# cs2mosa/Heterogeneous-MOE-for-Diffusion-models

Measured on AMD Instinct MI355X. Metric: denoise-steps/sec (fwd+bwd) on 4x32x32 latents, higher is better.
Workload: dtype bf16

## Files before the change

heterogeneous-moe-for-diffusion-models_amd/csrc/pbwd.hip:

```cpp
#include "common.h"
#include "conv_args.h"
#include "hdmoe.h"

namespace {

struct PbwArgs {
  const bf16* x; const bf16* dy; const bf16* wd; bf16* dx; float* G[HDMOE_MAX_GROUPS]; const int* seg;
  int ngroups, N, I, O, upw;
  long HW, wdstride;
  float alpha;
};
typedef __attribute__((ext_vector_type(4))) short s16x4;
typedef __attribute__((address_space(3))) s16x4* lds_p4;

DEVI bool pbw_slot(const PbwArgs& a, int slot, int& g, long& p0, long& p1, long& u0, long& u1) {
  for (g = 0; g < a.ngroups; ++g) {
    const long r0 = a.seg ? a.seg[g] : 0, r1 = a.seg ? a.seg[g + 1] : a.N;
    p0 = r0 * a.HW; p1 = r1 * a.HW;
    const long units = p1 > p0 ? (p1 - p0 + 63) >> 6 : 0;
    const long nch = (units + a.upw - 1) / a.upw;
    if (slot < nch) { u0 = (long)slot * a.upw; u1 = u0 + a.upw < units ? u0 + a.upw : units; return true; }
    slot -= (int)nch;
  }
  return false;
}

template <int OT, int IT>
__global__ __launch_bounds__(256) void pw_bwd_kernel(PbwArgs a) {
  constexpr int WB = (OT + IT) * 4096, T = OT * IT;
  extern __shared__ __attribute__((aligned(1024))) unsigned char lds[];
  const int tid = threadIdx.x, lane = tid & 63, wave = tid >> 6;
  int g; long p0, p1, u0, u1;
  if (!pbw_slot(a, blockIdx.x, g, p0, p1, u0, u1)) return;
  const bf16* X = a.x;
  const bf16* DY = a.dy;
  bf16* DX = a.dx;
  unsigned char* mine = lds + wave * WB;
  const int r = lane & 31, h = lane >> 5;
  bf16x8 wfr[IT][OT][2];
  {
    const bf16* WD = a.wd + (long)g * a.wdstride;
#pragma unroll
    for (int u = 0; u < IT; ++u)
#pragma unroll
      for (int t = 0; t < OT; ++t)
#pragma unroll
        for (int k2 = 0; k2 < 2; ++k2) wfr[u][t][k2] = *reinterpret_cast<const bf16x8*>(WD + (long)(32 * u + r) * a.O + 32 * t + 16 * k2 + 8 * h);
  }
  uint4 sdy[4 * OT], sx[4 * IT];
  auto load = [&](long u) {
    const long pb = p0 + (u << 6);
#pragma unroll
    for (int k = 0; k < 4 * OT; ++k) {
      const int e = lane + 64 * k, q = e / (4 * OT), pc = e % (4 * OT);
      const long p = pb + q;
      sdy[k] = *reinterpret_cast<const uint4*>(DY + (p < p1 ? p : p0) * a.O + pc * 8);
    }
#pragma unroll
    for (int k = 0; k < 4 * IT; ++k) {
      const int e = lane + 64 * k, q = e / (4 * IT), pc = e % (4 * IT);
      const long p = pb + q;
      sx[k] = *reinterpret_cast<const uint4*>(X + (p < p1 ? p : p0) * a.I + pc * 8);
    }
#pragma unroll
    for (int k = 0; k < 4 * OT; ++k) if (pb + (lane + 64 * k) / (4 * OT) >= p1) sdy[k] = make_uint4(0, 0, 0, 0);
#pragma unroll
    for (int k = 0; k < 4 * IT; ++k) if (pb + (lane + 64 * k) / (4 * IT) >= p1) sx[k] = make_uint4(0, 0, 0, 0);
  };
  auto store = [&]() {
#pragma unroll
    for (int k = 0; k < 4 * OT; ++k) {
      const int e = lane + 64 * k, q = e / (4 * OT), pc = e % (4 * OT);
      *reinterpret_cast<uint4*>(mine + (pc >> 2) * 4096 + q * 64 + (pc & 3) * 16) = sdy[k];
    }
#pragma unroll
    for (int k = 0; k < 4 * IT; ++k) {
      const int e = lane + 64 * k, q = e / (4 * IT), pc = e % (4 * IT);
      *reinterpret_cast<uint4*>(mine + OT * 4096 + (pc >> 2) * 4096 + q * 64 + (pc & 3) * 16) = sx[k];
    }
  };
  const int q4 = (lane & 15) >> 2, col4 = (lane & 16) + 4 * (lane & 3);
  const int tlane = (8 * h + q4) * 64 + col4 * 2;
  auto tr2 = [&](const unsigned char* base) -> bf16x8 {
    const s16x4 lo = __builtin_amdgcn_ds_read_tr16_b64_v4i16((lds_p4)(base));
    const s16x4 hi = __builtin_amdgcn_ds_read_tr16_b64_v4i16((lds_p4)(base + 4 * 64));
    return __builtin_bit_cast(bf16x8, __builtin_shufflevector(lo, hi, 0, 1, 2, 3, 4, 5, 6, 7));
  };
  f32x16 acc[OT][IT];
#pragma unroll
  for (int t = 0; t < OT; ++t)
#pragma unroll
    for (int u = 0; u < IT; ++u) acc[t][u] = (f32x16)(0.f);
  auto wfence = [&]() {
    __builtin_amdgcn_fence(__ATOMIC_RELEASE, "wavefront");
    __builtin_amdgcn_wave_barrier();
    __builtin_amdgcn_fence(__ATOMIC_ACQUIRE, "wavefront");
  };
  const long iters = (u1 - u0 + 3) >> 2;
  if (u0 + wave < u1) load(u0 + wave);
  for (long it = 0; it < iters; ++it) {
    const long u = u0 + wave + 4 * it;
    const bool valid = u < u1;
    wfence();
    if (valid) store();
    wfence();
    if (u + 4 < u1) load(u + 4);
    if (valid) {
#pragma unroll
      for (int ks = 0; ks < 4; ++ks) {
        bf16x8 fdy[OT], fx[IT];
#pragma unroll
        for (int t = 0; t < OT; ++t) fdy[t] = tr2(mine + t * 4096 + ks * 1024 + tlane);
#pragma unroll
        for (int v = 0; v < IT; ++v) fx[v] = tr2(mine + (OT + v) * 4096 + ks * 1024 + tlane);
#pragma unroll
        for (int t = 0; t < OT; ++t)
#pragma unroll
          for (int v = 0; v < IT; ++v) acc[t][v] = __builtin_amdgcn_mfma_f32_32x32x16_bf16(fdy[t], fx[v], acc[t][v], 0, 0, 0);
      }
      wfence();
#pragma unroll
      for (int hh = 0; hh < 2; ++hh) {
        f32x16 ax[IT];
#pragma unroll
        for (int v = 0; v < IT; ++v) ax[v] = (f32x16)(0.f);
#pragma unroll
        for (int t = 0; t < OT; ++t)
#pragma unroll
          for (int k2 = 0; k2 < 2; ++k2) {
            const bf16x8 d = *reinterpret_cast<const bf16x8*>(mine + t * 4096 + (32 * hh + r) * 64 + (2 * k2 + h) * 16);
#pragma unroll
            for (int v = 0; v < IT; ++v) ax[v] = __builtin_amdgcn_mfma_f32_32x32x16_bf16(wfr[v][t][k2], d, ax[v], 0, 0, 0);
          }
#pragma unroll
        for (int v = 0; v < IT; ++v)
#pragma unroll
          for (int q = 0; q < 4; ++q) {
            bf16x4 o4;
#pragma unroll
            for (int j = 0; j < 4; ++j) o4[j] = (bf16)(a.alpha * ax[v][4 * q + j]);
            *reinterpret_cast<bf16x4*>(mine + (OT + v) * 4096 + (32 * hh + r) * 64 + (8 * q + 4 * h) * 2) = o4;
          }
      }
      wfence();
      const long pb = p0 + (u << 6);
#pragma unroll
      for (int k = 0; k < 4 * IT; ++k) {
        const int e = lane + 64 * k, q = e / (4 * IT), pc = e % (4 * IT);
        const uint4 v = *reinterpret_cast<const uint4*>(mine + OT * 4096 + (pc >> 2) * 4096 + q * 64 + (pc & 3) * 16);
        if (pb + q < p1) *reinterpret_cast<uint4*>(DX + (pb + q) * a.I + pc * 8) = v;
      }
    }
  }
  float* red = reinterpret_cast<float*>(lds);
  auto put = [&](int s) {
#pragma unroll
    for (int t = 0; t < OT; ++t)
#pragma unroll
      for (int v = 0; v < IT; ++v)
#pragma unroll
        for (int reg = 0; reg < 16; ++reg) red[((s * T + t * IT + v) * 16 + reg) * 64 + lane] = acc[t][v][reg];
  };
  __syncthreads();
  if (wave >= 2) put(wave - 2);
  __syncthreads();
  if (wave < 2) {
#pragma unroll
    for (int t = 0; t < OT; ++t)
#pragma unroll
      for (int v = 0; v < IT; ++v)
#pragma unroll
        for (int reg = 0; reg < 16; ++reg) acc[t][v][reg] += red[((wave * T + t * IT + v) * 16 + reg) * 64 + lane];
  }
  __syncthreads();
  if (wave < 2) put(wave);
  __syncthreads();
  float* G = a.G[g];
  const int rot = (int)((blockIdx.x * 17u) % (unsigned)(T * 4)) * 256;
  for (int e0 = tid; e0 < T * 1024; e0 += 256) {
    const int e = (e0 + rot) % (T * 1024);
    const int l = e & 63, reg = (e >> 6) & 15, tu = e >> 10;
    const float v = red[(tu * 16 + reg) * 64 + l] + red[((T + tu) * 16 + reg) * 64 + l];
    const int o = 32 * (tu / IT) + acc_row(reg, l), i = 32 * (tu % IT) + (l & 31);
    atomicAdd(&G[(long)o * a.I + i], v);
  }
}

template <int OT, int IT>
int pbw_launch(const PbwArgs& a, unsigned slots, size_t lds, hipStream_t stream) {
  static unsigned long long attr = 0;
  if (hdmoe_first_on_device(attr)) { (void)hipFuncSetAttribute((const void*)pw_bwd_kernel<OT, IT>, hipFuncAttributeMaxDynamicSharedMemorySize, 160 * 1024); }
  hipLaunchKernelGGL((pw_bwd_kernel<OT, IT>), dim3(slots), dim3(256), lds, stream, a);
  return hdmoe_launch_status();
}

}

extern "C" int hdmoe_pw_bwd(const void* x, const void* dy, const void* wd, void* dx, float* const* G, const int* seg, int ngroups,
                            long wd_stride, int N, long HW, int Cin, int Cout, float alpha, int dtype, hipStream_t stream) {
  if (dtype != HDMOE_BF16 || Cin < 32 || Cout < 32 || Cin % 32 || Cout % 32 || Cin > 128 || Cout > 128) return 1;
  const int OT = Cout / 32, IT = Cin / 32;
  if (OT * IT > 8) return 1;
  if (!x || !dy || !wd || !dx || !G || ngroups < 1 || ngroups > HDMOE_MAX_GROUPS || N < 0 || HW < 0) return HDMOE_EINVAL;
  if ((((uintptr_t)x | (uintptr_t)dy | (uintptr_t)wd | (uintptr_t)dx) & 15) || wd_stride % 8 || wd_stride < (long)Cin * Cout) return 1;
  const long total = (long)N * HW;
  if (total == 0) return HDMOE_OK;
  if (total >= (1l << 40)) return 1;
  PbwArgs a;
  a.x = (const bf16*)x; a.dy = (const bf16*)dy; a.wd = (const bf16*)wd; a.dx = (bf16*)dx; a.seg = seg;
  a.ngroups = ngroups; a.N = N; a.HW = HW; a.I = Cin; a.O = Cout; a.wdstride = wd_stride; a.alpha = alpha;
  for (int g = 0; g < HDMOE_MAX_GROUPS; ++g) {
    a.G[g] = G[g < ngroups ? g : 0];
    if (!a.G[g]) return HDMOE_EINVAL;
  }
  const size_t stage = (size_t)4 * (OT + IT) * 4096, red = (size_t)2 * OT * IT * 4096;
  const size_t lds = stage > red ? stage : red;
  const long target = OT + IT <= 3 ? 512 : 256;
  const long units = (total + 63) / 64 + ngroups;
  long upw = (units + target - 1) / target;
  upw = (upw + 3) / 4 * 4;
  if (upw > (1l << 24)) return 1;
  a.upw = (int)upw;
  const long slots = units / upw + ngroups + 1;
  if (slots >= (1l << 31)) return 1;
  hdmoe_count_selection(HDMOE_SEL_PW_BWD);
  int rc = 1;
  conv_pick<1, 2, 3, 4>(OT, [&](auto Ot) { conv_pick<1, 2, 3, 4>(IT, [&](auto It) {
    constexpr int O = decltype(Ot)::value, I = decltype(It)::value;
    if constexpr (O * I <= 8) rc = pbw_launch<O, I>(a, (unsigned)slots, lds, stream);
  }); });
  return rc;
}
```

heterogeneous-moe-for-diffusion-models_amd/hdmoe_hip/ops.py:

```python
from __future__ import annotations

import ctypes
import functools
import math
from typing import Optional, Sequence, Tuple, Union

import torch

from . import bank as _bank
from ._lib import dtype_code_cast
from ._lib import BF16, _int_array, call, dtype_code, lib

Tensor = torch.Tensor

F32S = 2
ROUTE_CONV6S = 6


def _c(t: Optional[Tensor]) -> Optional[Tensor]:
    if t is None:
        return None
    return t if t.is_contiguous() else t.contiguous()


# ... 325 lines not shown
        return _fused_bwd(bank, ent, self.label, self.name, x, dy, ent.wd, dx, self.mid, ws, self.tail, self.defer, self.stats)


def _kxk_bwd_plan(L: _ConvLayer, seg, policy: str, stats: tuple, kernel: str, film: bool = False, gn_in=(None, None, 0)) -> _BwdPlan:
    geom, defer = (L.N, L.H, L.W, L.I, L.O, L.khs, L.kws, L.pts, L.pts, L.alpha), (seg, L.G, L.N, L.H, L.W, L.I, L.O, L.dtc, L.khs)
    if L.dtc != F32S:
        return _BwdPlan("hdmoe_conv_bwd6", L.dtc, policy, (seg, L.G, L.wdstride, *geom), (L.dtc,), defer, stats,
                        lambda: L.record(seg, 2.0, name=kernel, dtype="bfloat16"), film)
    return _BwdPlan("hdmoe_conv_bwd6s", F32S, policy, (seg, L.G, L.wdstride, L.G * L.wdstride, *geom), (*gn_in, 1 if TRUNK_BWD_BF16 else 0), defer, stats,
                    lambda: L.record(seg, 2.0, name=kernel, dtype="bfloat16" if TRUNK_BWD_BF16 else "split_bf16"))


def _conv_bwd_plan(L: _ConvLayer, seg, need_dx: bool, ones6: bool, device) -> Optional[_BwdPlan]:
    same = not L.ones and L.Ho == L.H and L.Wo == L.W and L.Cphys == L.I
    conv6 = need_dx and _prof_ok() and same and L.khs == L.kws
    if conv6 and L.dtc == BF16 and set(L.khs) == {3, 5}:
        return _kxk_bwd_plan(L, seg, "arena", ("bwd6",), "bwd6_kernel", film=True)
    if conv6 and L.split and set(L.khs) == {3}:
        return _kxk_bwd_plan(L, seg, "arena", ("bwd6s",), "bwd6s_kernel")
    if ones6:
        def scratch():
            S = torch.empty((L.G, L.H, L.W, L.O), dtype=torch.float32, device=device)
            g32 = [_zeros((kh * kw, L.O, L.Cphys), torch.float32, device) for kh, kw in zip(L.khs, L.kws)]
            return (S, g32, seg, L.G, L.wdstride, L.N, L.H, L.W, L.Cphys, L.O, L.Opad, L.khs, L.alpha)
        return _BwdPlan("hdmoe_conv6_ones_bwd", L.dtc, "stream", scratch, (L.dtc,), None, (),
                        lambda: L.record(seg, 2.0 if need_dx else 1.0, name="conv6 dgrad + wgrad6 (ones-channel layer)", dtype="bfloat16"))
    if need_dx and _prof_ok() and same and L.dtc == BF16 and all(k == 1 for k in L.khs + L.kws):
        return _BwdPlan("hdmoe_pw_bwd", L.dtc, None, (seg, L.G, L.wdstride, L.N, L.H * L.W, L.I, L.O, L.alpha), (L.dtc,), None, ("pbwd",),
                        lambda: L.record(seg, 2.0, name="pw_bwd_kernel", dtype="bfloat16"))
    return None


def _fused_bwd(bank, ent, label, name, x, dy, wd, dx, mid, ws, tail, defer, stats) -> bool:
    wsargs = () if ws is None else (ws, ws.numel() * 4)
    if _timed("fused", label, name, x, dy, wd, dx, list(ent.G), *mid, *wsargs, *tail) != 0:
        return False
    if defer is not None:
        seg, *shape = defer
        bank.defer_w6(ent.G, seg, ws, *shape, ent=ent)
    else:
        bank.note_backward(ent)
    for k in stats:
        STATS[k] += 1
    return True


def _wgrad(x, dy, Gs, seg, G, N, H, W, Ho, Wo, I, Cphys, O, ones, khs, kws, pts, split=False, bank=None):
    def rec(w6=None):
        if w6:
            return lambda: _conv_record(x, seg, N, Ho * Wo, O, I, khs, kws, "split_bf16" if split else None, wgrad_name=w6)
        return lambda: _conv_record(x, seg, N, Ho * Wo, O, I, khs, kws, wgrad_name=_kernel_label(_route(
            "hdmoe_conv_wgrad_route", 34, N, H, W, Ho, Wo, I, Cphys, O, 1, ones, G, seg is not None, khs, kws, pts, pts, _dt(x),
            x.data_ptr() % 16 == 0 and dy.data_ptr() % 16 == 0), x, wgrad=True))
    w6 = "wgrad6_kernel<split>" if split else "wgrad6_kernel"
    if (x.dtype == torch.bfloat16 or split) and not ones and Ho == H and Wo == W and Cphys == I:
        dtc = F32S if split else _dt(x)
        kib = _w6_kib(G, N, H, W, I, O, khs, kws, dtc)
        ws = _w6_workspace("arena", x.device, kib) if bank is not None and _prof_ok() else None
        if ws is not None:
            if _timed("conv_wgrad", rec(w6 + " (deferred reduce)"), "hdmoe_conv_wgrad6", x, dy, Gs, seg, G, N, H, W, I, O, khs, kws, pts, pts, ws, ws.numel() * 4,
                      dtc, 1) == 0:
                bank.defer_w6(Gs, seg, ws, G, N, H, W, I, O, dtc, khs)
                STATS["w6_defer"] += 1
                return
        ws = _w6_workspace("stream", x.device, kib)
        if ws is not None:
            if _timed("conv_wgrad", rec(w6 + " (+ reduce)"), "hdmoe_conv_wgrad6", x, dy, Gs, seg, G, N, H, W, I, O, khs, kws, pts, pts, ws, ws.numel() * 4, dtc, 0) == 0:
                return
    _timed("conv_wgrad", rec(), "hdmoe_conv_wgrad", x, dy, Gs, seg, G, N, H, W, Ho, Wo, I, Cphys, O, 1, 1 if ones else 0, khs, kws, pts, pts, _dt(x))


_ConvCall = _collections.namedtuple("_ConvCall", "G gain_val alpha beta ones training normalize split res_raw out film")


class _MPConvFn(torch.autograd.Function):

    @staticmethod
    def forward(ctx, x, res, seg, c: _ConvCall, *tensors):
        G, gain_val, alpha, beta, ones, training, normalize, split = c.G, c.gain_val, c.alpha, c.beta, c.ones, c.training, c.normalize, c.split
        weights, gains = tensors[:G], list(tensors[G:]) or None
        ctx.film = getattr(x, "_film_rec", None) if FILM_DGRAD and x.is_contiguous() else None
        if ctx.film is not None:
            ctx.film.register()
        x = _c(x)
        N, H, W, Cphys = x.shape
        O, I = int(weights[0].shape[0]), int(weights[0].shape[1])
        khs = [_kernel_hw(w)[0] for w in weights]
        kws = [_kernel_hw(w)[1] for w in weights]
        pts = [(kw - 1) // 2 for kw in kws]
        Hos = {H + (kw - 1) - kh + 1 for kh, kw in zip(khs, kws)}
        if len(Hos) != 1:
            raise ValueError("grouped conv: all groups must produce the same output size")
        if any(w.shape[0] != O or w.shape[1] != I for w in weights):
            raise ValueError("grouped conv: all groups must share (out_channels, in_channels)")
        if I != Cphys + (1 if ones else 0):
            raise RuntimeError(f"MP_Conv: input has {Cphys} channels, weight expects {I}")
        Ho, Wo = Hos.pop(), W
        Ipad = (I + 15) // 16 * 16
        Opad = (O + 15) // 16 * 16
        taps = max(a * b for a, b in zip(khs, kws))
        wstride, wdstride = taps * O * Ipad, taps * I * Opad
        wdt, planes, dtc = (torch.bfloat16, 2, F32S) if split else (x.dtype, 1, _dt(x))
        L = ctx.layer = _ConvLayer(G, N, H, W, Ho, Wo, Cphys, I, O, Ipad, Opad, khs, kws, pts, wstride, wdstride, dtc, gain_val, alpha, beta, ones,
                               normalize, split, c.res_raw, res is not None)
        ent = None
        if _bank.ACTIVE is not None and gains is None:
            ent = _bank.ACTIVE.lookup(weights, "split" if split else x.dtype, gain_val, alpha, normalize)
        if ent is not None:
            wf, wd = ent.wf, ent.wd
        else:
            wf = torch.empty(planes * G * wstride, dtype=wdt, device=x.device)
            wd = torch.empty(planes * G * wdstride, dtype=wdt, device=x.device) if ctx.needs_input_grad[0] else None
            call("hdmoe_wprep_fwd", list(weights), gains, gain_val, khs, kws, G, O, I, Ipad, Opad, wf, wstride, wd, wdstride,
                 1 if normalize else 0, 1 if training else 0, 1, dtc)
            if training and normalize:
                _bank.note_weights_changed()
        ctx.wd, ctx.ent, ctx.bank = wd, ent, (_bank.ACTIVE if ent is not None else None)
        bank16 = c.out is None and ent is not None and not split and res is None and x.dtype == torch.bfloat16 and Ho == H and Wo == W
        ones_dom = bank16 and ones and ONES6 and _prof_ok() and khs == kws
        film_dom = bank16 and c.film is not None and not ones and PROFILE is None and Cphys == I
        y = c.out if c.out is not None else torch.empty((N, Ho, Wo, O), dtype=x.dtype, device=x.device)
        gb = torch.empty((G, H, W, O), dtype=torch.float32, device=x.device) if ones_dom else None
        hbuf = torch.empty_like(y) if film_dom else None
        ctx.ones6 = False
        if c.out is not None:
            pass
        elif ones_dom and _timed("fused", lambda: L.record(seg, 1.0, name="conv6_bf16_kernel (ones-channel layer)", dtype="bfloat16"),
                                 "hdmoe_conv6_ones_fwd", x, wf, y, gb, alpha, seg, G, wstride, N, H, W, Cphys, O, Ipad, khs, dtc) == 0:
            ctx.ones6 = True
            STATS["ones6"] += 1
        elif film_dom and call("hdmoe_conv_fwd_film", x, wf, y, hbuf, c.film.emb, c.film.seed, step_counter(x.device), c.film.p, alpha, seg, G, wstride,
                               N, H, W, I, O, khs, kws, pts, pts, dtc) == 0:
            c.film.h = hbuf
        else:
            args = (x, wf, y, _c(res), alpha, beta,
                    seg, G, wstride, N, H, W, Ho, Wo, I, Cphys, Ipad, O, O, 1, 1 if ones else 0, khs, kws, pts, pts, dtc)
            _timed("conv_fwd", lambda: _fwd_record(*args), "hdmoe_conv_fwd", *args)
        ctx.save_for_backward(x, seg, *tensors)
        return y

    @staticmethod
    def backward(ctx, dy):
        x, seg, *tensors = ctx.saved_tensors
        L, nig = ctx.layer, ctx.needs_input_grad
        weights, gains = tensors[:L.G], list(tensors[L.G:]) or None
        dy = _c(dy)
        need_gain = gains is not None and any(nig[4 + L.G:])
        need_w = any(nig[4:4 + L.G]) or need_gain
        fused, dx = _conv_fused_bwd(ctx, L, x, dy, seg, nig[0]) if need_w and ctx.ent is not None else (False, None)
        if nig[0] and not fused:
            dx = _conv_dgrad(L, x, dy, ctx.wd, seg)
        dres = None
        if L.has_res and nig[1]:
            if L.res_raw or L.beta == 1.0:
                dres = dy
            else:
                dres = torch.empty_like(dy)
                call("hdmoe_axpby", dres, dy, None, L.beta, 0.0, dy.numel(), _dt(dy))
        dws, dgs = _conv_wgrad(ctx, L, x, dy, seg, weights, gains, need_gain) if need_w and not fused else ([None] * L.G, [None] * len(gains or ()))
        return (dx, dres, None, None, *dws, *dgs)


def _conv_fused_bwd(ctx, L: _ConvLayer, x, dy, seg, need_dx: bool):
    rec = ctx.film
    if rec is not None:
        rec.clear()
    plan = _conv_bwd_plan(L, seg, need_dx, ctx.ones6, x.device)
    ws = plan.workspace(L, x.device) if plan is not None and plan.policy is not None else None
    if plan is None or (ws is None and plan.policy is not None):
        return False, None
    if callable(plan.mid):
        plan = plan._replace(mid=plan.mid())
    dx = torch.empty_like(x) if need_dx else None
    fused = False
    if plan.film and rec is not None and FILM_DGRAD and need_dx and rec.sole_consumer(x):
        de = torch.empty(rec.e.shape, dtype=torch.float32, device=x.device)
        fused = plan._replace(name="hdmoe_conv_bwd6_film", tail=(rec.u, rec.e, rec.mask, de, rec.p, plan.dtc),
                              label=lambda: dict(plan.label(), name="bwd7_kernel (FiLM epilogue)")).launch(ctx.bank, ctx.ent, x, dy, dx, ws)
        if fused:
            rec.offer(dx, de)
            STATS["film_dgrad"] += 1
    fused = fused or plan.launch(ctx.bank, ctx.ent, x, dy, dx, ws)
    return fused, dx if fused else None


def _conv_dgrad(L: _ConvLayer, x, dy, wd, seg) -> Tensor:
    dx = torch.empty_like(x)
    pt_d = [kh - 1 - p for kh, p in zip(L.khs, L.pts)]
    pl_d = [kw - 1 - p for kw, p in zip(L.kws, L.pts)]
    args = (dy, wd, dx, None, L.alpha, 0.0,
            seg, L.G, L.wdstride, L.N, L.Ho, L.Wo, L.H, L.W, L.O, L.O, L.Opad, L.I, L.Cphys, 1, 0, L.khs, L.kws, pt_d, pl_d, L.dtc)
    _timed("conv_fwd", lambda: _fwd_record(*args), "hdmoe_conv_fwd", *args)
    return dx


def _conv_wgrad(ctx, L: _ConvLayer, x, dy, seg, weights, gains, need_gain: bool):
    G, O, I = L.G, L.O, L.I
    geom = (seg, G, L.N, L.H, L.W, L.Ho, L.Wo, I, L.Cphys, O, L.ones, L.khs, L.kws, L.pts, L.split)
    dgs = [None] * len(gains or ())
    if ctx.ent is not None:
        _wgrad(x, dy, ctx.ent.G, *geom, bank=ctx.bank)
        ctx.bank.note_backward(ctx.ent)
        return [None] * G, dgs
    sizes = [kh * kw * O * I for kh, kw in zip(L.khs, L.kws)]
    Gs = list(torch.zeros(sum(sizes), dtype=torch.float32, device=x.device).split(sizes))
    _wgrad(x, dy, Gs, *geom)
    dws = [torch.empty_like(w) for w in weights]
    if need_gain:
        dgs = [torch.zeros((), dtype=torch.float32, device=x.device) for _ in range(G)]
    call("hdmoe_wprep_bwd", list(weights), gains, L.gain_val, Gs, dws, dgs if need_gain else None, L.khs, L.kws, G, O, I, 1 if L.normalize else 0)
    if L.alpha != 1.0:
        for d in dws + [d for d in dgs if d is not None]:
            call("hdmoe_axpby", d, d, None, L.alpha, 0.0, d.numel(), 0)
    return dws, dgs



class _StridedConvFn(torch.autograd.Function):

    @staticmethod
    def forward(ctx, x, w, gain, stride, training):
        x = _c(x)
        N, H, W, C = x.shape
        O, I, kh, kw = (int(v) for v in w.shape)
        if I != C:
            raise RuntimeError(f"MP_Conv: input has {C} channels, weight expects {I}")
        pad = kw // 2
        Ho, Wo = (H + 2 * pad - kh) // stride + 1, (W + 2 * pad - kw) // stride + 1
        Ipad = (I + 15) // 16 * 16
        wf = torch.empty(kh * kw * O * Ipad, dtype=x.dtype, device=x.device)
        call("hdmoe_wprep_fwd", [w], None, float(gain), [kh], [kw], 1, O, I, Ipad, 16, wf, wf.numel(), None, 0, 1, 1 if training else 0, 1, _dt(x))
        if training:
            _bank.note_weights_changed()
        y = torch.empty((N, Ho, Wo, O), dtype=x.dtype, device=x.device)
        call("hdmoe_conv_fwd", x, wf, y, None, 1.0, 0.0, None, 1, wf.numel(), N, H, W, Ho, Wo, I, I, Ipad, O, O, stride, 0, [kh], [kw], [pad], [pad], _dt(x))
        ctx.save_for_backward(x, w)
        ctx.meta = (float(gain), stride, pad, Ho, Wo)
        return y

    @staticmethod
    def backward(ctx, dy):
        x, w = ctx.saved_tensors
        gain, stride, pad, Ho, Wo = ctx.meta
        if ctx.needs_input_grad[0]:
            raise NotImplementedError("MP_Conv(stride > 1): the input gradient is not implemented (no reference model uses a strided MP_Conv)")
        N, H, W, C = x.shape
        O, I, kh, kw = (int(v) for v in w.shape)
        dw = None
        if ctx.needs_input_grad[1]:
            Gs = [_zeros((kh * kw, O, I), torch.float32, x.device)]
            call("hdmoe_conv_wgrad", x, _c(dy), Gs, None, 1, N, H, W, Ho, Wo, I, I, O, stride, 0, [kh], [kw], [pad], [pad], _dt(x))
            dw = torch.empty_like(w)
            call("hdmoe_wprep_bwd", [w], None, gain, Gs, [dw], None, [kh], [kw], 1, O, I, 1)
        return None, dw, None, None, None


def mp_conv_strided(x: Tensor, w: Tensor, gain: float, stride: int, training: bool = False) -> Tensor:
    (w,) = f32_params([w])
    return _StridedConvFn.apply(x, w, float(gain), int(stride), bool(training))


def _split_ok(N: int, H: int, W: int, C: int, ws) -> bool:
    if any(w.ndim != 4 for w in ws):
        return False
    O, khs, kws = int(ws[0].shape[0]), [int(w.shape[2]) for w in ws], [int(w.shape[3]) for w in ws]
    pts = [(k - 1) // 2 for k in kws]
# ... 586 lines not shown
        x, s = ctx.saved_tensors
        g = _c(g)
        rows = x.shape[0]
        L = x.numel() // rows
        dx = torch.empty_like(x) if ctx.needs_input_grad[0] else None
        ds = _zeros(s.shape, s.dtype, s.device, ctx.pool_ok) if ctx.needs_input_grad[1] else None
        call("hdmoe_scale_rows_bwd", dx, ds, g, x, s, rows, L, _dt(x))
        return dx, ds


def scale_rows(x: Tensor, s: Tensor) -> Tensor:
    return _ScaleRowsFn.apply(x, s)


class _Cat2Fn(torch.autograd.Function):
    @staticmethod
    def forward(ctx, a, b, wa, wb):
        a = _c(a); b = _c(b)
        Ca, Cb = a.shape[-1], b.shape[-1]
        rows = a.numel() // Ca
        out = torch.empty((*a.shape[:-1], Ca + Cb), dtype=a.dtype, device=a.device)
        call("hdmoe_cat2_fwd", out, a, b, wa, wb, Ca, Cb, rows, _dt(a))
        ctx.meta = (wa, wb, a.shape, b.shape)
        return out

    @staticmethod
    def backward(ctx, g):
        wa, wb, sa, sb = ctx.meta
        g = _c(g)
        da = torch.empty(sa, dtype=g.dtype, device=g.device)
        db = torch.empty(sb, dtype=g.dtype, device=g.device)
        call("hdmoe_cat2_bwd", da, db, g, wa, wb, sa[-1], sb[-1], da.numel() // sa[-1], _dt(g))
        return da, db, None, None


def mp_cat(a: Tensor, b: Tensor, t: float = 0.5) -> Tensor:
    na, nb = a.shape[-1], b.shape[-1]
    c = math.sqrt((na + nb) / ((1.0 - t) ** 2 + t ** 2))
    return _Cat2Fn.apply(a, b, c * (1.0 - t) / math.sqrt(na), c * t / math.sqrt(nb))


class _SiluBranchFn(torch.autograd.Function):

    @staticmethod
    def forward(ctx, x, gx_scale):
        ctx.set_materialize_grads(False)
        x = _c(x)
        h = torch.empty_like(x)
        call("hdmoe_mp_silu_fwd", h, x, x.numel(), _dt(x))
        ctx.save_for_backward(x)
        ctx.sx = float(gx_scale)
        return x.view(x.shape), h

    @staticmethod
    def backward(ctx, gx, gh):
        (x,) = ctx.saved_tensors
        if gh is None:
            if gx is None or ctx.sx == 1.0:
                return gx, None
            dx = torch.empty_like(x)
            call("hdmoe_axpby", dx, _c(gx), None, ctx.sx, 0.0, dx.numel(), _dt(dx))
            return dx, None
        gh = _c(gh)
        dx = torch.empty_like(x)
        if gx is None:
            call("hdmoe_mp_silu_bwd", dx, gh, x, x.numel(), _dt(x))
        else:
            call("hdmoe_mp_silu_bwd_add", dx, gh, x, _c(gx), ctx.sx, x.numel(), _dt(x))
        return dx, None


class _CatSiluFn(torch.autograd.Function):

    @staticmethod
    def forward(ctx, a, b, wa, wb):
        ctx.set_materialize_grads(False)
        a = _c(a); b = _c(b)
        Ca, Cb = a.shape[-1], b.shape[-1]
        out = torch.empty((*a.shape[:-1], Ca + Cb), dtype=a.dtype, device=a.device)
        h = torch.empty_like(out)
        call("hdmoe_cat2_silu_fwd", out, h, a, b, wa, wb, Ca, Cb, a.numel() // Ca, _dt(a))
        ctx.save_for_backward(out)
        ctx.meta = (wa, wb, a.shape, b.shape)
        return out, h

    @staticmethod
    def backward(ctx, gcat, gh):
        (out,) = ctx.saved_tensors
        wa, wb, sa, sb = ctx.meta
        da = torch.empty(sa, dtype=out.dtype, device=out.device)
        db = torch.empty(sb, dtype=out.dtype, device=out.device)
        if gh is None:
            if gcat is None:
                return None, None, None, None
            call("hdmoe_cat2_bwd", da, db, _c(gcat), wa, wb, sa[-1], sb[-1], da.numel() // sa[-1], _dt(out))
        else:
            call("hdmoe_cat2_silu_bwd", da, db, None if gcat is None else _c(gcat), _c(gh), out, wa, wb, sa[-1], sb[-1], da.numel() // sa[-1], _dt(out))
        return da, db, None, None


def _vec_ok(*ts) -> bool:
    return all(t.shape[-1] % (8 if t.dtype == torch.bfloat16 else 4) == 0 and t.dtype in (torch.bfloat16, torch.float32) for t in ts)


def silu_branch(x: Tensor, gx_scale: float = 1.0):
    if _vec_ok(x) and x.numel() % 8 == 0:
        return _SiluBranchFn.apply(x, float(gx_scale))
    x, xh = fanout(x, 2)
    if gx_scale != 1.0:
        x = affine_grad(x, gx_scale)
    return x, mp_silu(xh)


class _GradScaleFn(torch.autograd.Function):
    @staticmethod
    def forward(ctx, x, s):
        ctx.s = s
        return x.view(x.shape)

    @staticmethod
    def backward(ctx, g):
        g = _c(g)
        dx = torch.empty_like(g)
        call("hdmoe_axpby", dx, g, None, ctx.s, 0.0, g.numel(), _dt(g))
        return dx, None


def affine_grad(x: Tensor, s: float) -> Tensor:
    return _GradScaleFn.apply(x, float(s))


def mp_cat_silu(a: Tensor, b: Tensor, t: float = 0.5):
    if not (_vec_ok(a, b) and a.dtype == b.dtype):
        return silu_branch(mp_cat(a, b, t))
    na, nb = a.shape[-1], b.shape[-1]
    c = math.sqrt((na + nb) / ((1.0 - t) ** 2 + t ** 2))
    return _CatSiluFn.apply(a, b, c * (1.0 - t) / math.sqrt(na), c * t / math.sqrt(nb))


class _ResampleFn(torch.autograd.Function):
    @staticmethod
    def forward(ctx, x, mode):
        x = _c(x)
        N, H, W, C = x.shape
        ctx.mode = mode
        if mode == "down":
            out = torch.empty((N, H // 2, W // 2, C), dtype=x.dtype, device=x.device)
            call("hdmoe_pool2", out, x, N, H // 2, W // 2, C, 0.25, _dt(x))
        else:
            out = torch.empty((N, H * 2, W * 2, C), dtype=x.dtype, device=x.device)
            call("hdmoe_upsample2", out, x, N, H * 2, W * 2, C, 1.0, _dt(x))
        return out

    @staticmethod
    def backward(ctx, g):
        g = _c(g)
        N, H, W, C = g.shape
        if ctx.mode == "down":
            dx = torch.empty((N, H * 2, W * 2, C), dtype=g.dtype, device=g.device)
            call("hdmoe_upsample2", dx, g, N, H * 2, W * 2, C, 0.25, _dt(g))
        else:
            dx = torch.empty((N, H // 2, W // 2, C), dtype=g.dtype, device=g.device)
            call("hdmoe_pool2", dx, g, N, H // 2, W // 2, C, 1.0, _dt(g))
        return dx, None


class _FirResampleFn(torch.autograd.Function):

    @staticmethod
    def forward(ctx, x, taps, mode):
        x = _c(x)
        N, H, W, C = x.shape
        L = len(taps)
        pad = (L - 1) // 2
# ... 1525 lines not shown
```

include/hdmoe.h:

```cpp
#ifndef HDMOE_H
#define HDMOE_H
#ifdef __cplusplus
extern "C" {
#endif

#ifndef HDMOE_OK
#define HDMOE_OK 0
#define HDMOE_EINVAL (-1)
#define HDMOE_EDTYPE (-2)
#define HDMOE_ELAUNCH (-3)
#define HDMOE_F32 0
#define HDMOE_BF16 1
#define HDMOE_F16 3
#define HDMOE_F32S 2
#define HDMOE_MAX_GROUPS 8
#endif

typedef void* hdmoe_stream_t;
#ifdef __HIPCC__
#define HS hipStream_t
#else
#define HS hdmoe_stream_t
#endif

int hdmoe_version(void);

int hdmoe_wprep_fwd(float* const* w_raw, const float* const* gain_ptr, float gain_val, const int* kh, const int* kw,
                    int ngroups, int O, int I, int Ipad, int Opad, void* wf, long wf_stride, void* wd, long wd_stride,
                    int normalize, int mutate, int flip, int dtype, HS stream);
int hdmoe_wprep_bwd(const float* const* w_raw, const float* const* gain_ptr, float gain_val, const float* const* G,
                    float* const* dw, float* const* dgain, const int* kh, const int* kw, int ngroups, int O, int I,
                    int normalize, HS stream);
int hdmoe_conv_fwd(const void* x, const void* w, void* y, const void* res, float alpha, float beta, const int* seg,
                   int ngroups, long wstride, int N, int H, int W, int Ho, int Wo, int Cin, int Cphys, int Ipad, int Cout,
                   int Cstore, int stride, int ones, const int* kh, const int* kw, const int* pt, const int* pl, int dtype,
                   HS stream);
int hdmoe_conv_wgrad(const void* x, const void* dy, float* const* G, const int* seg, int ngroups, int N, int H, int W,
                     int Ho, int Wo, int Cin, int Cphys, int Cout, int stride, int ones, const int* kh, const int* kw,
                     const int* pt, const int* pl, int dtype, HS stream);

int hdmoe_conv_wgrad6_ws_kib(int ngroups, int N, int H, int W, int Cin, int Cout, const int* kh, const int* kw, int dtype);
int hdmoe_conv_wgrad6(const void* x, const void* dy, float* const* G, const int* seg, int ngroups, int N, int H, int W, int Cin,
                      int Cout, const int* kh, const int* kw, const int* pt, const int* pl, void* ws, long ws_bytes, int dtype,
                      int defer, HS stream);
int hdmoe_conv_bwd6(const void* x, const void* dy, const void* wd, void* dx, float* const* G, const int* seg, int ngroups,
                    long wd_stride, int N, int H, int W, int Cin, int Cout, const int* kh, const int* kw, const int* pt,
                    const int* pl, float alpha, void* ws, long ws_bytes, int dtype, HS stream);
int hdmoe_conv_bwd6_film(const void* x, const void* dy, const void* wd, void* dx, float* const* G, const int* seg, int ngroups,
                         long wd_stride, int N, int H, int W, int Cin, int Cout, const int* kh, const int* kw, const int* pt,
                         const int* pl, float alpha, void* ws, long ws_bytes, const void* film_u, const float* film_e,
                         const unsigned char* film_mask, float* film_de, float film_p, int dtype, HS stream);
int hdmoe_pw_bwd(const void* x, const void* dy, const void* wd, void* dx, float* const* G, const int* seg, int ngroups,
                 long wd_stride, int N, long HW, int Cin, int Cout, float alpha, int dtype, HS stream);
int hdmoe_conv_bwd6s(const void* x, const void* dy, const void* wd, void* dx, float* const* G, const int* seg, int ngroups,
                     long wd_stride, long wd_plane, int N, int H, int W, int Cin, int Cout, const int* kh, const int* kw,
                     const int* pt, const int* pl, float alpha, void* ws, long ws_bytes, const float* in_scale, const float* in_shift,
                     int in_relu, int hi_only, HS stream);
int hdmoe_conv_fwd_split_gn(const void* x, const void* w, void* y, const float* in_scale, const float* in_shift, int in_relu,
                            float* stats_ws, long wstride, long wplane, int N, int H, int W, int Cin, int Cout, float alpha, HS stream);
int hdmoe_conv_fwd_film(const void* x, const void* w, void* y, void* h, const float* e, unsigned long long seed,
                        const unsigned long long* seed_dev, float p, float alpha, const int* seg, int ngroups, long wstride, int N, int H, int W,
                        int Cin, int Cout, const int* kh, const int* kw, const int* pt, const int* pl, int dtype, HS stream);
int hdmoe_conv_split_stats_slots(int H, int W, int Cout);
int hdmoe_gn1_finalize(float* scale, float* shift, float* mean, float* rstd, const float* ws, const float* gamma, const float* beta,
                       int N, int slots, int C, long count, float eps, HS stream);
int hdmoe_gn1_relu_mean(float* out, const float* y, const float* scale, const float* shift, int N, long S, int C, HS stream);
int hdmoe_gn1_finalize_relu_mean(float* out, float* scale, float* shift, float* mean, float* rstd, const float* y, const float* ws,
                                 const float* gamma, const float* beta, int N, int slots, long S, int C, float eps, HS stream);
int hdmoe_gn1_finalize_relu_mean_pq(float* out, float* scale, float* shift, float* mean, float* rstd, float* pcnt, float* qsum, const float* y,
                                    const float* ws, const float* gamma, const float* beta, int N, int slots, long S, int C, float eps, HS stream);
int hdmoe_conv_wgrad6_reduce_batch(float* const* G, const int* const* seg, float* const* ws, const int* dims, int n, HS stream);

int hdmoe_conv6_debug_stamps(void* buf);

enum {
  HDMOE_SEL_CONV7_32 = 0,
  HDMOE_SEL_CONV7_16 = 1,
  HDMOE_SEL_CONV6 = 2,
  HDMOE_SEL_CONV6S = 3,
  HDMOE_SEL_BWD7_32 = 4,
  HDMOE_SEL_BWD7_32_WGRAD8 = 5,
  HDMOE_SEL_BWD7_32_WGRAD7 = 6,
  HDMOE_SEL_BWD7_16_OT1 = 7,
  HDMOE_SEL_BWD7_16_OT2 = 8,
  HDMOE_SEL_BWD6 = 9,
  HDMOE_SEL_BWD6S = 10,
  HDMOE_SEL_WGRAD6_DIRECT = 11,
  HDMOE_SEL_WGRAD6_DEFER = 12,
  HDMOE_SEL_BLK6 = 13,
  HDMOE_SEL_WGRAD8_C11 = 14,
  HDMOE_SEL_WGRAD8_C12 = 15,
  HDMOE_SEL_WGRAD8_C21 = 16,
  HDMOE_SEL_WGRAD8_C22 = 17,
  HDMOE_SEL_PW_BWD = 18,
  HDMOE_SEL_RELAYOUT_TILED = 19,
  HDMOE_SEL_COMBINE_FWD_VEC = 20,
  HDMOE_SEL_COMBINE_BWD_VEC = 21,
  HDMOE_SEL_FILM_DGRAD = 22,
  HDMOE_SEL_ROW_WINDOW = 23,
  HDMOE_SEL_COUNT = 24
};
int hdmoe_kernel_selections(long long* counts, int n, int reset);

enum {
  HDMOE_ROUTE_CONV_FWD = 0,
  HDMOE_ROUTE_CONV_FWD2 = 1,
  HDMOE_ROUTE_CONV_FWD3 = 2,
  HDMOE_ROUTE_CONV_FWD5 = 3,
  HDMOE_ROUTE_CONV_CONV7 = 4,
  HDMOE_ROUTE_CONV_CONV6 = 5,
  HDMOE_ROUTE_CONV_CONV6S = 6,
  HDMOE_ROUTE_CONV_KGEMM = 7,
  HDMOE_ROUTE_CONV_GLIN = 8,
  HDMOE_ROUTE_CONV_NONE = 9,
  HDMOE_ROUTE_CONV_ROWLIN = 10,
  HDMOE_ROUTE_WGRAD_V2 = 0,
  HDMOE_ROUTE_WGRAD_V1 = 1,
  HDMOE_ROUTE_WGRAD_SWG = 2,
  HDMOE_ROUTE_WGRAD_TOWG = 3,
  HDMOE_ROUTE_WGRAD_LWG = 4
};
int hdmoe_conv_fwd_route(int* route, int N, int H, int W, int Ho, int Wo, int Cin, int Cphys, int Ipad, int Cout, int Cstore, int stride, int ones,
                         int ngroups, int has_seg, int has_res, long wstride, const int* kh, const int* kw, const int* pt, const int* pl,
                         int dtype, int aligned16);
int hdmoe_conv_generic_route(int* route, int N, int H, int W, int Ho, int Wo, int Cin, int Cphys, int Ipad, int Cout, int Cstore, int stride,
                             int ones, int ngroups, const int* kh, const int* kw, int dtype, int aligned16);
int hdmoe_conv7_min_images(void);
int hdmoe_conv_wgrad_route(int* route, int N, int H, int W, int Ho, int Wo, int Cin, int Cphys, int Cout, int stride, int ones, int ngroups,
                           int has_seg, const int* kh, const int* kw, const int* pt, const int* pl, int dtype, int aligned16);

int hdmoe_wbank_desc_bytes(void);
int hdmoe_wbank_prep(const void* descs, const int* rows, int nrows, int mutate, HS stream);
int hdmoe_wbank_bwd(const void* descs, const int* rows, int nrows, HS stream);

int hdmoe_axpby(void* out, const void* x, const void* y, float a, float b, long n, int dtype, HS stream);
int hdmoe_sum_n(void* out, const void* const* srcs, const float* src_scale, int n, long nelem, int dtype, HS stream);
int hdmoe_affine(void* out, const void* x, float a, float c, long n, int dtype, HS stream);
int hdmoe_mul(void* out, const void* x, const void* y, long n, int dtype, HS stream);
int hdmoe_sched_pick(float* sigma, const double* t, const int* idx, int off, HS stream);
int hdmoe_idx_advance(int* idx, HS stream);
int hdmoe_heun_euler(float* xn, const float* xh, const float* den, const double* t, const int* idx, long n,
                     const float* x0, const float* noise, const float* mask, HS stream);
int hdmoe_heun_correct(float* out, const float* xh, const float* den, const float* xn, const float* den2, const double* t, const int* idx, long n,
                       const float* x0, const float* noise, const float* mask, HS stream);
int hdmoe_known_blend(void* x, const void* x0, const void* noise, const float* mask, float s, long n, int dtype, HS stream);
int hdmoe_dpm2m_step(float* x_out, const float* x, const float* den, float* den_prev, const double* t, const int* idx, const int* i0, long n,
                     const float* x0, const float* noise, const float* mask, HS stream);
int hdmoe_heun_churn(float* x_hat, const float* x, float* sigma, double* t_hat, const double* t, const int* idx, const unsigned long long* seed,
                     double gamma_cap, double s_min, double s_max, double s_noise, long n, HS stream);
int hdmoe_heun_euler_hat(float* xn, const float* xh, const float* den, const double* t, const int* idx, const double* t_hat, long n,
                         const float* x0, const float* noise, const float* mask, HS stream);
int hdmoe_heun_correct_hat(float* out, const float* xh, const float* den, const float* xn, const float* den2, const double* t, const int* idx,
                           const double* t_hat, long n, const float* x0, const float* noise, const float* mask, HS stream);
int hdmoe_dpm2m_sde_step(float* x_out, const float* x, const float* den, float* den_prev, const double* t, const int* idx, const int* i0, long n,
                         const float* x0, const float* noise, const float* mask, float eta, float s_noise, const unsigned long long* seed,
                         HS stream);
int hdmoe_exp_rate(float* out, int blocks, int iters, HS stream);
int hdmoe_cast(void* out, const void* x, long n, int dt_in, int dt_out, HS stream);
int hdmoe_fir_resample(void* y, const void* x, const float* taps, int L, int pad, float scale, int up, int N, int H, int W, int Ho, int Wo, int C,
                       int dtype, HS stream);
int hdmoe_mp_silu_fwd(void* out, const void* x, long n, int dtype, HS stream);
int hdmoe_mp_silu_bwd(void* dx, const void* dy, const void* x, long n, int dtype, HS stream);
int hdmoe_mp_silu_bwd_add(void* dx, const void* dy, const void* x, const void* gx, float sx, long n, int dtype, HS stream);
int hdmoe_cat2_silu_fwd(void* out, void* out_h, const void* a, const void* b, float wa, float wb, int Ca, int Cb, long rows,
                        int dtype, HS stream);
int hdmoe_cat2_silu_bwd(void* da, void* db, const void* gcat, const void* gh, const void* xcat, float wa, float wb, int Ca,
                        int Cb, long rows, int dtype, HS stream);
int hdmoe_sigmoid_fwd(void* out, const void* x, float a, long n, int dtype, HS stream);
int hdmoe_sigmoid_bwd(void* dx, const void* dy, const void* y, float a, long n, int dtype, HS stream);
int hdmoe_film_silu_fwd(void* out, const void* u, const float* e, int N, long HW, int C, int dtype, HS stream);
int hdmoe_film_silu_bwd(void* du, float* de, const void* da, const void* u, const float* e, int N, long HW, int C,
                        int dtype, HS stream);
int hdmoe_film_silu_drop_fwd(void* out, const void* u, const float* e, int N, long HW, int C, unsigned long long seed,
                             const unsigned long long* seed_dev, float p, int dtype, HS stream);
int hdmoe_film_silu_drop_bwd(void* du, float* de, const void* da, const void* u, const float* e, int N, long HW, int C,
                             unsigned long long seed, const unsigned long long* seed_dev, float p, int dtype, HS stream);
int hdmoe_film_silu_drop_fwd_mask(void* out, unsigned char* mask, const void* u, const float* e, int N, long HW, int C,
                                  unsigned long long seed, const unsigned long long* seed_dev, float p, int dtype, HS stream);
int hdmoe_film_silu_mask_bwd(void* du, float* de, const void* da, const void* u, const float* e, const unsigned char* mask, int N,
                             long HW, int C, float p, int dtype, HS stream);
int hdmoe_scale_rows_fwd(void* out, const void* x, const float* s, long rows, long L, int dtype, HS stream);
int hdmoe_scale_rows_bwd(void* dx, float* ds, const void* dy, const void* x, const float* s, long rows, long L,
                         int dtype, HS stream);
// ... 227 lines not shown
```

Measured before the change: 90.19.

## Fuse mp_cat+SiLU backward into pointwise conv backward tail via deferred launch

Defers the pointwise conv backward when its input came from the mp_cat_silu op, then runs it inside the cat's backward. There the dx tile is combined in LDS with the SiLU gradient term and weights, and da/db are written directly. This removes the dx round trip through global memory and a separate cat/silu backward kernel. In exchange it adds autograd-ordering bookkeeping with runtime checks, extra LDS staging per wave and narrower MFMA grouping for large tiles.

```diff
diff --git a/heterogeneous-moe-for-diffusion-models_amd/csrc/pbwd.hip b/heterogeneous-moe-for-diffusion-models_amd/csrc/pbwd.hip
--- a/heterogeneous-moe-for-diffusion-models_amd/csrc/pbwd.hip
+++ b/heterogeneous-moe-for-diffusion-models_amd/csrc/pbwd.hip
@@ -9,6 +9,9 @@
   int ngroups, N, I, O, upw;
   long HW, wdstride;
   float alpha;
+  const bf16* gh; bf16* da; bf16* db;
+  int Ca;
+  float wa, wb;
 };
 typedef __attribute__((ext_vector_type(4))) short s16x4;
 typedef __attribute__((address_space(3))) s16x4* lds_p4;
@@ -25,9 +28,9 @@
   return false;
 }
 
-template <int OT, int IT>
+template <int OT, int IT, bool CAT>
 __global__ __launch_bounds__(256) void pw_bwd_kernel(PbwArgs a) {
-  constexpr int WB = (OT + IT) * 4096, T = OT * IT;
+  constexpr int WB = (OT + IT) * 4096 + (CAT ? IT * 2048 : 0), T = OT * IT, VG = CAT && T >= 6 ? 1 : IT;
   extern __shared__ __attribute__((aligned(1024))) unsigned char lds[];
   const int tid = threadIdx.x, lane = tid & 63, wave = tid >> 6;
   int g; long p0, p1, u0, u1;
@@ -47,7 +50,35 @@
 #pragma unroll
         for (int k2 = 0; k2 < 2; ++k2) wfr[u][t][k2] = *reinterpret_cast<const bf16x8*>(WD + (long)(32 * u + r) * a.O + 32 * t + 16 * k2 + 8 * h);
   }
-  uint4 sdy[4 * OT], sx[4 * IT];
+  uint4 sdy[4 * OT], sx[4 * IT], sgh[CAT ? 2 * IT : 1];
+  auto load_gh = [&](long u, int hh) {
+    const long pb = p0 + (u << 6) + 32 * hh;
+#pragma unroll
+    for (int k = 0; k < (CAT ? 2 * IT : 0); ++k) {
+      const int e = lane + 64 * k, q = e / (4 * IT), pc = e % (4 * IT);
+      const long p = pb + q;
+      sgh[k] = *reinterpret_cast<const uint4*>(a.gh + (p < p1 ? p : p0) * a.I + pc * 8);
+    }
+  };
+  auto cat_tail = [&](long u, int hh) {
+    const unsigned char* stg = mine + (OT + IT) * 4096;
+    const long pb = p0 + (u << 6) + 32 * hh;
+    const int Cb = a.I - a.Ca;
+#pragma unroll
+    for (int k = 0; k < 2 * IT; ++k) {
+      const int e = lane + 64 * k, q = e / (4 * IT), pc = e % (4 * IT);
+      const bf16x8 dv = *reinterpret_cast<const bf16x8*>(stg + (pc >> 2) * 2048 + q * 64 + (pc & 3) * 16);
+      const bf16x8 xv = *reinterpret_cast<const bf16x8*>(mine + (OT + (pc >> 2)) * 4096 + (32 * hh + q) * 64 + (pc & 3) * 16);
+      const bf16x8 gv = __builtin_bit_cast(bf16x8, sgh[CAT ? k : 0]);
+      const int c = pc * 8;
+      const bool first = c < a.Ca;
+      const float wgt = first ? a.wa : a.wb;
+      float f[8];
+#pragma unroll
+      for (int j = 0; j < 8; ++j) f[j] = ((float)dv[j] + (float)gv[j] * mp_silu_grad_f((float)xv[j])) * wgt;
+      if (pb + q < p1) vstore<bf16>(first ? a.da + (pb + q) * a.Ca + c : a.db + (pb + q) * Cb + (c - a.Ca), f);
+    }
+  };
   auto load = [&](long u) {
     const long pb = p0 + (u << 6);
 #pragma unroll
@@ -106,6 +137,7 @@
     wfence();
     if (u + 4 < u1) load(u + 4);
     if (valid) {
+      load_gh(u, 0);
 #pragma unroll
       for (int ks = 0; ks < 4; ++ks) {
         bf16x8 fdy[OT], fx[IT];
@@ -118,37 +150,49 @@
 #pragma unroll
           for (int v = 0; v < IT; ++v) acc[t][v] = __builtin_amdgcn_mfma_f32_32x32x16_bf16(fdy[t], fx[v], acc[t][v], 0, 0, 0);
       }
-      wfence();
+      if constexpr (!CAT) wfence();
 #pragma unroll
       for (int hh = 0; hh < 2; ++hh) {
-        f32x16 ax[IT];
-#pragma unroll
-        for (int v = 0; v < IT; ++v) ax[v] = (f32x16)(0.f);
-#pragma unroll
-        for (int t = 0; t < OT; ++t)
-#pragma unroll
-          for (int k2 = 0; k2 < 2; ++k2) {
-            const bf16x8 d = *reinterpret_cast<const bf16x8*>(mine + t * 4096 + (32 * hh + r) * 64 + (2 * k2 + h) * 16);
-#pragma unroll
-            for (int v = 0; v < IT; ++v) ax[v] = __builtin_amdgcn_mfma_f32_32x32x16_bf16(wfr[v][t][k2], d, ax[v], 0, 0, 0);
-          }
-#pragma unroll
-        for (int v = 0; v < IT; ++v)
-#pragma unroll
-          for (int q = 0; q < 4; ++q) {
-            bf16x4 o4;
-#pragma unroll
-            for (int j = 0; j < 4; ++j) o4[j] = (bf16)(a.alpha * ax[v][4 * q + j]);
-            *reinterpret_cast<bf16x4*>(mine + (OT + v) * 4096 + (32 * hh + r) * 64 + (8 * q + 4 * h) * 2) = o4;
-          }
+#pragma unroll
+        for (int v0 = 0; v0 < IT; v0 += VG) {
+          f32x16 ax[VG];
+#pragma unroll
+          for (int v = 0; v < VG; ++v) ax[v] = (f32x16)(0.f);
+#pragma unroll
+          for (int t = 0; t < OT; ++t)
+#pragma unroll
+            for (int k2 = 0; k2 < 2; ++k2) {
+              const bf16x8 d = *reinterpret_cast<const bf16x8*>(mine + t * 4096 + (32 * hh + r) * 64 + (2 * k2 + h) * 16);
+#pragma unroll
+              for (int v = 0; v < VG; ++v) ax[v] = __builtin_amdgcn_mfma_f32_32x32x16_bf16(wfr[v0 + v][t][k2], d, ax[v], 0, 0, 0);
+            }
+#pragma unroll
+          for (int v = 0; v < VG; ++v)
+#pragma unroll
+            for (int q = 0; q < 4; ++q) {
+              bf16x4 o4;
+#pragma unroll
+              for (int j = 0; j < 4; ++j) o4[j] = (bf16)(a.alpha * ax[v][4 * q + j]);
+              if constexpr (CAT) *reinterpret_cast<bf16x4*>(mine + (OT + IT) * 4096 + (v0 + v) * 2048 + r * 64 + (8 * q + 4 * h) * 2) = o4;
+              else *reinterpret_cast<bf16x4*>(mine + (OT + v0 + v) * 4096 + (32 * hh + r) * 64 + (8 * q + 4 * h) * 2) = o4;
+            }
+        }
+        if constexpr (CAT) {
+          wfence();
+          cat_tail(u, hh);
+          if (hh == 0) load_gh(u, 1);
+          wfence();
+        }
       }
-      wfence();
-      const long pb = p0 + (u << 6);
-#pragma unroll
-      for (int k = 0; k < 4 * IT; ++k) {
-        const int e = lane + 64 * k, q = e / (4 * IT), pc = e % (4 * IT);
-        const uint4 v = *reinterpret_cast<const uint4*>(mine + OT * 4096 + (pc >> 2) * 4096 + q * 64 + (pc & 3) * 16);
-        if (pb + q < p1) *reinterpret_cast<uint4*>(DX + (pb + q) * a.I + pc * 8) = v;
+      if constexpr (!CAT) {
+        wfence();
+        const long pb = p0 + (u << 6);
+#pragma unroll
+        for (int k = 0; k < 4 * IT; ++k) {
+          const int e = lane + 64 * k, q = e / (4 * IT), pc = e % (4 * IT);
+          const uint4 v = *reinterpret_cast<const uint4*>(mine + OT * 4096 + (pc >> 2) * 4096 + q * 64 + (pc & 3) * 16);
+          if (pb + q < p1) *reinterpret_cast<uint4*>(DX + (pb + q) * a.I + pc * 8) = v;
+        }
       }
     }
   }
@@ -186,34 +230,34 @@
   }
 }
 
-template <int OT, int IT>
+template <int OT, int IT, bool CAT>
 int pbw_launch(const PbwArgs& a, unsigned slots, size_t lds, hipStream_t stream) {
   static unsigned long long attr = 0;
-  if (hdmoe_first_on_device(attr)) { (void)hipFuncSetAttribute((const void*)pw_bwd_kernel<OT, IT>, hipFuncAttributeMaxDynamicSharedMemorySize, 160 * 1024); }
-  hipLaunchKernelGGL((pw_bwd_kernel<OT, IT>), dim3(slots), dim3(256), lds, stream, a);
+  if (hdmoe_first_on_device(attr)) { (void)hipFuncSetAttribute((const void*)pw_bwd_kernel<OT, IT, CAT>, hipFuncAttributeMaxDynamicSharedMemorySize, 160 * 1024); }
+  hipLaunchKernelGGL((pw_bwd_kernel<OT, IT, CAT>), dim3(slots), dim3(256), lds, stream, a);
   return hdmoe_launch_status();
 }
 
-}
-
-extern "C" int hdmoe_pw_bwd(const void* x, const void* dy, const void* wd, void* dx, float* const* G, const int* seg, int ngroups,
-                            long wd_stride, int N, long HW, int Cin, int Cout, float alpha, int dtype, hipStream_t stream) {
+int pbw_run(PbwArgs& a, bool cat, const void* x, const void* dy, const void* wd, float* const* G, const int* seg, int ngroups, long wd_stride,
+            int N, long HW, int Cin, int Cout, float alpha, int dtype, hipStream_t stream) {
   if (dtype != HDMOE_BF16 || Cin < 32 || Cout < 32 || Cin % 32 || Cout % 32 || Cin > 128 || Cout > 128) return 1;
   const int OT = Cout / 32, IT = Cin / 32;
   if (OT * IT > 8) return 1;
-  if (!x || !dy || !wd || !dx || !G || ngroups < 1 || ngroups > HDMOE_MAX_GROUPS || N < 0 || HW < 0) return HDMOE_EINVAL;
-  if ((((uintptr_t)x | (uintptr_t)dy | (uintptr_t)wd | (uintptr_t)dx) & 15) || wd_stride % 8 || wd_stride < (long)Cin * Cout) return 1;
+  if (cat && (a.Ca < 8 || a.Ca > Cin - 8 || a.Ca % 8)) return 1;
+  const bool outs = cat ? a.gh && a.da && a.db : a.dx != nullptr;
+  if (!x || !dy || !wd || !outs || !G || ngroups < 1 || ngroups > HDMOE_MAX_GROUPS || N < 0 || HW < 0) return HDMOE_EINVAL;
+  const uintptr_t ptrs = (uintptr_t)x | (uintptr_t)dy | (uintptr_t)wd | (uintptr_t)a.dx | (uintptr_t)a.gh | (uintptr_t)a.da | (uintptr_t)a.db;
+  if ((ptrs & 15) || wd_stride % 8 || wd_stride < (long)Cin * Cout) return 1;
   const long total = (long)N * HW;
   if (total == 0) return HDMOE_OK;
   if (total >= (1l << 40)) return 1;
-  PbwArgs a;
-  a.x = (const bf16*)x; a.dy = (const bf16*)dy; a.wd = (const bf16*)wd; a.dx = (bf16*)dx; a.seg = seg;
+  a.x = (const bf16*)x; a.dy = (const bf16*)dy; a.wd = (const bf16*)wd; a.seg = seg;
   a.ngroups = ngroups; a.N = N; a.HW = HW; a.I = Cin; a.O = Cout; a.wdstride = wd_stride; a.alpha = alpha;
   for (int g = 0; g < HDMOE_MAX_GROUPS; ++g) {
     a.G[g] = G[g < ngroups ? g : 0];
     if (!a.G[g]) return HDMOE_EINVAL;
   }
-  const size_t stage = (size_t)4 * (OT + IT) * 4096, red = (size_t)2 * OT * IT * 4096;
+  const size_t stage = (size_t)4 * ((OT + IT) * 4096 + (cat ? IT * 2048 : 0)), red = (size_t)2 * OT * IT * 4096;
   const size_t lds = stage > red ? stage : red;
   const long target = OT + IT <= 3 ? 512 : 256;
   const long units = (total + 63) / 64 + ngroups;
@@ -223,11 +267,29 @@
   a.upw = (int)upw;
   const long slots = units / upw + ngroups + 1;
   if (slots >= (1l << 31)) return 1;
-  hdmoe_count_selection(HDMOE_SEL_PW_BWD);
+  hdmoe_count_selection(cat ? HDMOE_SEL_PW_CAT_SILU_BWD : HDMOE_SEL_PW_BWD);
   int rc = 1;
   conv_pick<1, 2, 3, 4>(OT, [&](auto Ot) { conv_pick<1, 2, 3, 4>(IT, [&](auto It) {
     constexpr int O = decltype(Ot)::value, I = decltype(It)::value;
-    if constexpr (O * I <= 8) rc = pbw_launch<O, I>(a, (unsigned)slots, lds, stream);
+    if constexpr (O * I <= 8) rc = cat ? pbw_launch<O, I, true>(a, (unsigned)slots, lds, stream) : pbw_launch<O, I, false>(a, (unsigned)slots, lds, stream);
   }); });
   return rc;
 }
+
+}
+
+extern "C" int hdmoe_pw_bwd(const void* x, const void* dy, const void* wd, void* dx, float* const* G, const int* seg, int ngroups,
+                            long wd_stride, int N, long HW, int Cin, int Cout, float alpha, int dtype, hipStream_t stream) {
+  PbwArgs a = {};
+  a.dx = (bf16*)dx;
+  return pbw_run(a, false, x, dy, wd, G, seg, ngroups, wd_stride, N, HW, Cin, Cout, alpha, dtype, stream);
+}
+
+extern "C" int hdmoe_pw_cat_silu_bwd(const void* x, const void* dy, const void* wd, const void* gh, float* const* G, const int* seg,
+                                     int ngroups, long wd_stride, int N, long HW, int Cin, int Cout, float alpha, void* da, void* db,
+                                     float wa, float wb, int Ca, int Cb, int dtype, hipStream_t stream) {
+  if (Ca < 0 || Cb < 0 || Cb % 8 || Ca + Cb != Cin) return 1;
+  PbwArgs a = {};
+  a.gh = (const bf16*)gh; a.da = (bf16*)da; a.db = (bf16*)db; a.Ca = Ca; a.wa = wa; a.wb = wb;
+  return pbw_run(a, true, x, dy, wd, G, seg, ngroups, wd_stride, N, HW, Cin, Cout, alpha, dtype, stream);
+}
diff --git a/heterogeneous-moe-for-diffusion-models_amd/hdmoe_hip/ops.py b/heterogeneous-moe-for-diffusion-models_amd/hdmoe_hip/ops.py
--- a/heterogeneous-moe-for-diffusion-models_amd/hdmoe_hip/ops.py
+++ b/heterogeneous-moe-for-diffusion-models_amd/hdmoe_hip/ops.py
@@ -431,6 +431,9 @@
         ctx.film = getattr(x, "_film_rec", None) if FILM_DGRAD and x.is_contiguous() else None
         if ctx.film is not None:
             ctx.film.register()
+        ctx.cat = getattr(x, "_cat_rec", None) if CAT_SKIP_FUSED and x.is_contiguous() else None
+        if ctx.cat is not None:
+            ctx.cat.register()
         x = _c(x)
         N, H, W, Cphys = x.shape
         O, I = int(weights[0].shape[0]), int(weights[0].shape[1])
@@ -496,7 +499,11 @@
         dy = _c(dy)
         need_gain = gains is not None and any(nig[4 + L.G:])
         need_w = any(nig[4:4 + L.G]) or need_gain
-        fused, dx = _conv_fused_bwd(ctx, L, x, dy, seg, nig[0]) if need_w and ctx.ent is not None else (False, None)
+        fused, dx = (False, None)
+        if need_w and ctx.ent is not None:
+            fused, dx = _cat_defer(ctx, L, x, dy, seg) if ctx.cat is not None and nig[0] else (False, None)
+            if not fused:
+                fused, dx = _conv_fused_bwd(ctx, L, x, dy, seg, nig[0])
         if nig[0] and not fused:
             dx = _conv_dgrad(L, x, dy, ctx.wd, seg)
         dres = None
@@ -531,6 +538,58 @@
             STATS["film_dgrad"] += 1
     fused = fused or plan.launch(ctx.bank, ctx.ent, x, dy, dx, ws)
     return fused, dx if fused else None
+
+
+CAT_SKIP_FUSED = True
+
+
+class _CatRec:
+    __slots__ = ("taken", "pending")
+
+    def __init__(self):
+        self.taken, self.pending = 0, None
+
+    def register(self) -> None:
+        self.taken += 1
+
+
+class _CatPending:
+    __slots__ = ("plan", "L", "x", "dy", "seg", "dx", "wd", "ent", "bank")
+
+    def __init__(self, plan, L, x, dy, seg, dx, wd, ent, bank):
+        self.plan, self.L, self.x, self.dy, self.seg, self.dx, self.wd, self.ent, self.bank = plan, L, x, dy, seg, dx, wd, ent, bank
+
+    def launch_cat(self, gh, da, db, wa, wb) -> bool:
+        plan = self.plan
+        cat = plan._replace(name="hdmoe_pw_cat_silu_bwd", tail=(da, db, wa, wb, da.shape[-1], db.shape[-1], plan.dtc), stats=("pbwd_cat",),
+                            label=lambda: dict(plan.label(), name="pw_bwd_kernel<CAT> (mp_cat + mp_silu backward in the slice tail)"))
+        return cat.launch(self.bank, self.ent, self.x, self.dy, gh, None)
+
+    def launch_alone(self) -> Tensor:
+        if self.plan.launch(self.bank, self.ent, self.x, self.dy, self.dx, None):
+            return self.dx
+        dx = _conv_dgrad(self.L, self.x, self.dy, self.wd, self.seg)
+        _conv_wgrad(self, self.L, self.x, self.dy, self.seg, None, None, False)
+        return dx
+
+
+def _cat_defer(ctx, L: _ConvLayer, x, dy, seg):
+    rec = ctx.cat
+    rec.pending = None
+    if not (CAT_SKIP_FUSED and rec.taken == 1):
+        return False, None
+    plan = _conv_bwd_plan(L, seg, True, ctx.ones6, x.device)
+    if plan is None or plan.name != "hdmoe_pw_bwd":
+        return False, None
+    rec.pending = pend = _CatPending(plan, L, x, dy, seg, torch.empty_like(x), ctx.wd, ctx.ent, ctx.bank)
+
+    def check():
+        if rec.pending is pend:
+            rec.pending = None
+            raise RuntimeError("mp_cat_silu: the backward pass ended before the node that was to run the skip projection's backward "
+                               "(set ops.CAT_SKIP_FUSED = False)")
+    torch.autograd.Variable._execution_engine.queue_callback(check)
+    return True, pend.dx
 
 
 def _conv_dgrad(L: _ConvLayer, x, dy, wd, seg) -> Tensor:
@@ -1283,6 +1342,9 @@
         call("hdmoe_cat2_silu_fwd", out, h, a, b, wa, wb, Ca, Cb, a.numel() // Ca, _dt(a))
         ctx.save_for_backward(out)
         ctx.meta = (wa, wb, a.shape, b.shape)
+        ctx.rec = None
+        if CAT_SKIP_FUSED and out.dtype == torch.bfloat16 and out.ndim == 4 and _bank.ACTIVE is not None:
+            ctx.rec = out._cat_rec = _CatRec()
         return out, h
 
     @staticmethod
@@ -1291,6 +1353,16 @@
         wa, wb, sa, sb = ctx.meta
         da = torch.empty(sa, dtype=out.dtype, device=out.device)
         db = torch.empty(sb, dtype=out.dtype, device=out.device)
+        pend = None
+        if ctx.rec is not None:
+            pend, ctx.rec.pending = ctx.rec.pending, None
+        if pend is not None:
+            if gcat is None or gcat.data_ptr() != pend.dx.data_ptr() or gcat.shape != pend.dx.shape:
+                raise RuntimeError("mp_cat_silu: the concatenation fed a second consumer beside the pointwise layer that deferred its backward "
+                                   "(set ops.CAT_SKIP_FUSED = False)")
+            if gh is not None and pend.launch_cat(_c(gh), da, db, wa, wb):
+                return da, db, None, None
+            gcat = pend.launch_alone()
         if gh is None:
             if gcat is None:
                 return None, None, None, None
diff --git a/include/hdmoe.h b/include/hdmoe.h
--- a/include/hdmoe.h
+++ b/include/hdmoe.h
@@ -52,6 +52,9 @@
                          const unsigned char* film_mask, float* film_de, float film_p, int dtype, HS stream);
 int hdmoe_pw_bwd(const void* x, const void* dy, const void* wd, void* dx, float* const* G, const int* seg, int ngroups,
                  long wd_stride, int N, long HW, int Cin, int Cout, float alpha, int dtype, HS stream);
+int hdmoe_pw_cat_silu_bwd(const void* x, const void* dy, const void* wd, const void* gh, float* const* G, const int* seg, int ngroups,
+                          long wd_stride, int N, long HW, int Cin, int Cout, float alpha, void* da, void* db, float wa, float wb,
+                          int Ca, int Cb, int dtype, HS stream);
 int hdmoe_conv_bwd6s(const void* x, const void* dy, const void* wd, void* dx, float* const* G, const int* seg, int ngroups,
                      long wd_stride, long wd_plane, int N, int H, int W, int Cin, int Cout, const int* kh, const int* kw,
                      const int* pt, const int* pl, float alpha, void* ws, long ws_bytes, const float* in_scale, const float* in_shift,
@@ -98,7 +101,8 @@
   HDMOE_SEL_COMBINE_BWD_VEC = 21,
   HDMOE_SEL_FILM_DGRAD = 22,
   HDMOE_SEL_ROW_WINDOW = 23,
-  HDMOE_SEL_COUNT = 24
+  HDMOE_SEL_PW_CAT_SILU_BWD = 24,
+  HDMOE_SEL_COUNT = 25
 };
 int hdmoe_kernel_selections(long long* counts, int n, int reset);
 
```

Measured after the change: 91.43, median of 6. 1.01x the previous value.
